# Axe--/Visual-Question-Answering

Hardware: AMD Instinct MI355X
Metric: QA-pairs/sec (train step, attention model, K=1000) (higher is better)
Workload: dtype f32

## Files before the change

include/coattn.h:

```cpp
#ifndef COATTN_H
#define COATTN_H

#include <stddef.h>
#include <stdint.h>

#ifdef __cplusplus
extern "C" {
#endif

#define COATTN_F32 0
#define COATTN_BF16 1

#define COATTN_IMPL_AUTO 0
#define COATTN_IMPL_GENERAL 1
#define COATTN_IMPL_FUSED 2
#define COATTN_FLAG_BF16_PROJ 4
#define COATTN_FLAG_BF16_IN 8
#define COATTN_FLAG_EXACT3 16
#define COATTN_FLAG_SPLIT2 32
#define COATTN_FLAG_F16PAIR 64
#define COATTN_FLAG_FAST16 128
#define COATTN_FLAG_BILINEAR 256
typedef struct coattn_params {
  const void* W_v; const void* b_v;
// ... 145 lines not shown
                         const void* g_loss, const void* g_logits, void* const* dv, void* const* dq,
                         const coattn_head_param_grads* pg, int accumulate, void* ws, int B, int d, int mlp, int K,
                         int dtype, int flags, void* stream);

#define COATTN_LOSS_SOFT_CE 1
#define COATTN_LOSS_BCE 2
int coattn_soft_loss_forward(const void* logits, const void* ans_idx, const void* ans_score, int A, int kind,
                             void* loss, void* dlogits, void* ws, int B, int K, int dtype, void* stream);
int coattn_vqa_score(const void* logits, const void* ans_idx, const void* ans_score, int A,
                     void* pred, void* row_score, void* score_sum,
                     void* ws, int B, int K, int dtype, void* stream);
int coattn_head_forward_soft(const void* const* v, const void* const* q, const coattn_head_params* p,
                             const void* ans_idx, const void* ans_score, int A, int kind,
                             void* logits, void* loss, void* saved, int B, int d, int mlp, int K, int dtype, int flags,
                             void* stream);

typedef struct coattn_adam_tensor {
  void* p; const void* g; void* m; void* v; int64_t n;
} coattn_adam_tensor;
size_t coattn_adam_workspace_bytes(const coattn_adam_tensor* t, int n_tensors);
int coattn_adam_step(const coattn_adam_tensor* t, int n_tensors, int step, double lr, double beta1, double beta2,
                     double eps, double weight_decay, double max_grad_norm, void* norm_out, void* ws, size_t ws_bytes,
                     void* stream);

int coattn_bn_supported(int B, int H, int W, int C, int pool, int dtype);
size_t coattn_bn_workspace_bytes(int B, int H, int W, int C);
int coattn_bn_relu_pool_forward(const void* x, const void* gamma, const void* beta, const void* conv_bias,
                                void* running_mean, void* running_var, double momentum, double eps, void* y,
                                void* stats_out, void* ws, int B, int H, int W, int C, int pool, int relu, int dtype,
                                void* stream);

int coattn_relu_pool_forward(const void* x, void* y, int B, int H, int W, int C, int dtype, void* stream);


typedef struct coattn_gemm_desc {
  const void* A; const void* B; const void* Cin; void* C;
  const void* bias_n; const void* bias_m;
  int M, N, K, batch, inner, inner_total, ksplit, act;
  float beta;
  int64_t a_sm, a_sk, a_sz, a_si, a_mdiv, a_sdiv;
  int64_t b_sk, b_sn, b_sz, b_si;
  int64_t c_sm, c_sn, c_sz, c_mdiv, c_sdiv;
  int64_t cin_sm, cin_sn, cin_sz, cin_mdiv, cin_sdiv;
  const void* a_ptrs[8]; const void* b_ptrs[8]; void* c_ptrs[8]; const void* cin_ptrs[8];
  int ptr_by_inner; int b_imod;
  int kband_n; int kband_lo[3]; int kband_hi[3];
  float out_scale;
} coattn_gemm_desc;

int coattn_gemm_f32(const coattn_gemm_desc* g, void* stream);

size_t coattn_linear_workspace_bytes(int N, int K);
int coattn_linear_forward(const void* x, int64_t ld_x, const void* W, const void* bias, void* y, void* wimg,
                          int M, int N, int K, float out_scale, int flags, void* stream);

size_t coattn_linear_wgrad_workspace_bytes(int n_out, int n_in);
int coattn_linear_weight_grad(const void* dy, int64_t ld_dy, const void* x, int64_t ld_x, void* dW, void* ws, int M,
                              int n_out, int n_in, int accumulate, void* stream);

int coattn_gemm_bf16(const coattn_gemm_desc* g, void* stream);

int coattn_p2p_enable_peer(int peer_device);
int coattn_p2p_reduce_scatter(const void* const* peer_bufs, int world, int rank, int64_t shard_elems, float scale,
                              void* stream);
int coattn_p2p_all_gather(const void* const* peer_bufs, int world, int rank, int64_t shard_elems, void* stream);

// ... 5 lines not shown
```

visual-question-answering_amd/_lib.py:

```python
from __future__ import annotations

import ctypes as C
import os
import subprocess

_HERE = os.path.dirname(os.path.abspath(__file__))
LIB_PATH = os.environ.get("COATTN_LIB_PATH") or os.path.join(_HERE, "libcoattn_hip.so")
CSRC = os.path.join(_HERE, "csrc")

EXPORTS = ("coattn_version", "coattn_last_error", "coattn_fused_supported", "coattn_workspace_bytes",
           "coattn_forward", "coattn_attention_forward", "coattn_backward", "coattn_gemm_f32", "coattn_gemm_bf16",
           "coattn_phrase_workspace_bytes", "coattn_phrase_forward", "coattn_phrase_backward",
           "coattn_ce_workspace_bytes", "coattn_ce_forward", "coattn_linear_workspace_bytes", "coattn_linear_forward",
           "coattn_linear_wgrad_workspace_bytes", "coattn_linear_weight_grad",
           "coattn_head_workspace_bytes", "coattn_head_forward", "coattn_head_backward", "coattn_head_status",
           "coattn_ce_status", "coattn_p2p_enable_peer", "coattn_p2p_reduce_scatter", "coattn_p2p_all_gather",
           "coattn_profile_begin", "coattn_profile_end", "coattn_features_native", "coattn_status",
           "coattn_phrase_status", "coattn_status_accumulate", "coattn_phrase_status_accumulate", "coattn_infer",
           "coattn_forward_len", "coattn_infer_len", "coattn_attention_forward_len", "coattn_backward_len",
           "coattn_forward_maps", "coattn_forward_maps_len", "coattn_backward_maps", "coattn_backward_maps_len",
           "coattn_alt_workspace_bytes", "coattn_alt_forward", "coattn_alt_backward",
           "coattn_soft_loss_forward", "coattn_vqa_score", "coattn_head_forward_soft",
           "coattn_adam_workspace_bytes", "coattn_adam_step",
           "coattn_bn_supported", "coattn_bn_workspace_bytes", "coattn_bn_relu_pool_forward", "coattn_relu_pool_forward")

F32 = 0
BF16 = 1
IMPL_AUTO, IMPL_GENERAL, IMPL_FUSED = 0, 1, 2
FLAG_BF16_PROJ = 4
FLAG_BF16_IN = 8
FLAG_EXACT3 = 16
FLAG_SPLIT2 = 32
FLAG_F16PAIR = 64
FLAG_FAST16 = 128
LOSS_SOFT_CE, LOSS_BCE = 1, 2
MAX_ANSWERS = 16
LOSS_KINDS = {"soft_ce": LOSS_SOFT_CE, "bce": LOSS_BCE}
FLAG_BILINEAR = 256


def precision_flag(fast: bool) -> int:
    return FLAG_FAST16 if fast else 0


def default_fast() -> bool:
    return os.environ.get("VQA_PRECISION", "exact") == "fast"


class Params(C.Structure):
    _fields_ = [(n, C.c_void_p) for n in ("W_v", "b_v", "W_q", "b_q", "w_v", "c_v", "w_q", "c_q", "W_b", "b_b")]


class ParamGrads(C.Structure):
    _fields_ = [(n, C.c_void_p) for n in ("dW_v", "db_v", "dW_q", "db_q", "dw_v", "dc_v", "dw_q", "dc_q", "dW_b", "db_b")]


ALT_PARAM_NAMES = ("W_x1", "b_x1", "w_h1", "c_h1", "W_x2", "b_x2", "W_g2", "b_g2", "w_h2", "c_h2",
# ... 192 lines not shown
    lib.coattn_linear_workspace_bytes.restype = C.c_size_t
    lib.coattn_linear_forward.argtypes = ([C.c_void_p, C.c_int64] + [C.c_void_p] * 4 + [C.c_int] * 3
                                          + [C.c_float, C.c_int, C.c_void_p])
    lib.coattn_linear_wgrad_workspace_bytes.argtypes = [C.c_int, C.c_int]
    lib.coattn_linear_wgrad_workspace_bytes.restype = C.c_size_t
    lib.coattn_linear_weight_grad.argtypes = ([C.c_void_p, C.c_int64, C.c_void_p, C.c_int64, C.c_void_p, C.c_void_p]
                                              + [C.c_int] * 4 + [C.c_void_p])
    lib.coattn_ce_status.argtypes = [C.c_void_p, C.c_int, C.c_void_p]
    lib.coattn_status.argtypes = [C.c_void_p] + [C.c_int] * 6 + [C.c_void_p, C.POINTER(C.c_float)]
    lib.coattn_phrase_status.argtypes = [C.c_void_p] + [C.c_int] * 3 + [C.c_void_p, C.POINTER(C.c_float)]
    lib.coattn_status_accumulate.argtypes = [C.c_void_p] + [C.c_int] * 6 + [C.c_void_p, C.c_void_p]
    lib.coattn_phrase_status_accumulate.argtypes = [C.c_void_p] + [C.c_int] * 3 + [C.c_void_p, C.c_void_p]
    lib.coattn_p2p_enable_peer.argtypes = [C.c_int]
    lib.coattn_p2p_reduce_scatter.argtypes = [C.POINTER(C.c_void_p), C.c_int, C.c_int, C.c_int64, C.c_float, C.c_void_p]
    lib.coattn_p2p_all_gather.argtypes = [C.POINTER(C.c_void_p), C.c_int, C.c_int, C.c_int64, C.c_void_p]
    lib.coattn_profile_begin.argtypes = [C.c_void_p]
    lib.coattn_profile_end.argtypes = [C.POINTER(C.c_float), C.c_char_p, C.c_int, C.c_int]
    lib.coattn_features_native.argtypes = [C.c_void_p, C.c_int, C.c_int64, C.c_int64, C.c_int64, C.c_void_p,
                                           C.c_int, C.c_int, C.c_int, C.c_void_p]
    lib.coattn_head_status.argtypes = [C.c_void_p] + [C.c_int] * 4 + [C.c_void_p]
    lib.coattn_head_workspace_bytes.argtypes = [C.c_int] * 5 + [C.POINTER(C.c_size_t)] * 2
    lib.coattn_soft_loss_forward.argtypes = [C.c_void_p] * 3 + [C.c_int] * 2 + [C.c_void_p] * 3 + [C.c_int] * 3 + [C.c_void_p]
    lib.coattn_vqa_score.argtypes = [C.c_void_p] * 3 + [C.c_int] + [C.c_void_p] * 4 + [C.c_int] * 3 + [C.c_void_p]
    lib.coattn_adam_workspace_bytes.argtypes = [C.POINTER(AdamTensor), C.c_int]
    lib.coattn_adam_workspace_bytes.restype = C.c_size_t
    lib.coattn_adam_step.argtypes = ([C.POINTER(AdamTensor), C.c_int, C.c_int] + [C.c_double] * 6
                                     + [C.c_void_p, C.c_void_p, C.c_size_t, C.c_void_p])
    lib.coattn_bn_supported.argtypes = [C.c_int] * 6
    lib.coattn_bn_workspace_bytes.argtypes = [C.c_int] * 4
    lib.coattn_bn_workspace_bytes.restype = C.c_size_t
    lib.coattn_bn_relu_pool_forward.argtypes = ([C.c_void_p] * 6 + [C.c_double] * 2 + [C.c_void_p] * 3 + [C.c_int] * 7
                                                + [C.c_void_p])
    lib.coattn_relu_pool_forward.argtypes = [C.c_void_p] * 2 + [C.c_int] * 5 + [C.c_void_p]
    _lib = lib
    return lib


class RangeError(FloatingPointError):
    """An operand of the tolerance mode (FLAG_FAST16) left the exact range of its two FP16 pieces: the call's results are
    clamped, not within tolerance of the reference.  Use the exact mode (the modules' default; Trainer(precision="exact"))."""


F16_EXACT = 65504.0

_pending = []
_range_acc = {}


def note_status(kind: str, buf, dims, dev) -> None:
    import torch
    _pending.append((kind, buf, dims, dev, torch.cuda.current_stream(dev).cuda_stream))
    if not torch.cuda.is_current_stream_capturing():
        fold_range()


def _acc(dev):
    import torch
    key = dev.index if dev.index is not None else torch.cuda.current_device()
    a = _range_acc.get(key)
    if a is None:
        a = _range_acc[key] = torch.zeros(2, device=dev, dtype=torch.float32)
    return a


def fold_range() -> None:
    lib = load()
# ... 99 lines not shown
```

visual-question-answering_amd/csrc/api.hip:

```cpp
#include "common.h"
#include "fused.h"

#include <string.h>

static thread_local char g_err[512] = "";

void coattn_set_error(const char* fmt, ...) {
  va_list ap;
  va_start(ap, fmt);
  vsnprintf(g_err, sizeof(g_err), fmt, ap);
  va_end(ap);
}

extern "C" int coattn_version(void) { return 1400; }

namespace {
constexpr int kProfMax = 48;
struct Prof {
  bool on = false;
  int n = 0, created = 0;
  hipEvent_t ev[kProfMax + 1];
  const char* name[kProfMax];
};
thread_local Prof g_prof;
}

void prof_mark(hipStream_t s, const char* name) {
  Prof& p = g_prof;
  if (!p.on || p.n >= kProfMax) return;
  if (hipEventRecord(p.ev[p.n + 1], s) != hipSuccess) { p.on = false; return; }
  p.name[p.n++] = name;
}

extern "C" int coattn_profile_begin(void* stream) {
  Prof& p = g_prof;
  while (p.created <= kProfMax) {
    if (hipEventCreate(&p.ev[p.created]) != hipSuccess) { coattn_set_error("profile: hipEventCreate failed"); return -3; }
    ++p.created;
  }
  p.n = 0;
  if (hipEventRecord(p.ev[0], (hipStream_t)stream) != hipSuccess) { coattn_set_error("profile: hipEventRecord failed"); return -3; }
  p.on = true;
  return 0;
}

extern "C" int coattn_profile_end(float* us, char* names, int names_bytes, int max_marks) {
  Prof& p = g_prof;
// ... 818 lines not shown
```

visual-question-answering_amd/csrc/encoder.hip:

```cpp
#include <math.h>

#include "common.h"

namespace {

constexpr int kThreads = 256;
constexpr int kMaxStatBlocks = 2048;
constexpr int kPixelsPerStatBlock = 400;
constexpr int kMaxNormBlocks = 4096;
constexpr int kStatLoads = 8;

typedef double f64x2 __attribute__((ext_vector_type(2)));

inline int stat_blocks(int64_t pixels) {
  const int64_t g = pixels / kPixelsPerStatBlock;
  return g < 1 ? 1 : g > kMaxStatBlocks ? kMaxStatBlocks : (int)g;
}

inline size_t partial_bytes(int G, int C) { return (size_t)G * C * sizeof(f64x2); }

__global__ __launch_bounds__(kThreads) void bn_stats_partial_kernel(const f32x4* __restrict__ x, f64x2* __restrict__ partial,
                                                                    int64_t total4, int c4) {
  __shared__ double sh[8][kThreads];
  const int tid = threadIdx.x;
// ... 57 lines not shown
    const f64x2 p = partial[(int64_t)g * C + c];
    s += p.x;
    q += p.y;
  }
  sh[0][tid] = s;
  sh[1][tid] = q;
  for (int w = kThreads / 2; w >= 4; w >>= 1) {
    __syncthreads();
    if (tid < w) {
      s += sh[0][tid + w];
      q += sh[1][tid + w];
      sh[0][tid] = s;
      sh[1][tid] = q;
    }
  }
  if (tid >= 4) return;
  const double mean = s / count;
  double var = q / count - mean * mean;
  var = var < 0.0 ? 0.0 : var;
  const float mean_hi = (float)mean;
  ws_f[c] = mean_hi;
  ws_f[C + c] = (float)(mean - (double)mean_hi);
  ws_f[2 * C + c] = (float)((double)gamma[c] / sqrt(var + eps));
  ws_f[3 * C + c] = (float)var;
  const double bias = conv_bias ? (double)conv_bias[c] : 0.0;
  running_mean[c] = (float)((1.0 - momentum) * (double)running_mean[c] + momentum * (mean + bias));
  running_var[c] = (float)((1.0 - momentum) * (double)running_var[c] + momentum * (var * (count / (count - 1.0))));
  if (stats_out) {
    stats_out[c] = mean_hi;
    stats_out[C + c] = (float)var;
  }
}

struct Affine {
  float mean[4], lo[4], scale[4], beta[4];
};

__device__ __forceinline__ f32x4 affine(const f32x4 v, const Affine& a) {
  f32x4 t;
#pragma unroll
  for (int e = 0; e < 4; ++e) t[e] = fmaf((v[e] - a.mean[e]) - a.lo[e], a.scale[e], a.beta[e]);
  return t;
}
__device__ __forceinline__ f32x4 max_nan(const f32x4 a, const f32x4 b) {
  f32x4 m;
#pragma unroll
  for (int e = 0; e < 4; ++e) m[e] = (a[e] > b[e] || a[e] != a[e]) ? a[e] : b[e];
  return m;
}
__device__ __forceinline__ f32x4 relu_nan(const f32x4 a) {
  f32x4 r;
#pragma unroll
  for (int e = 0; e < 4; ++e) r[e] = a[e] < 0.f ? 0.f : a[e];
  return r;
}

template <bool POOL, bool AFFINE = true>
__global__ __launch_bounds__(kThreads) void bn_relu_pool_kernel(const f32x4* __restrict__ x, const float* __restrict__ ws_f,
                                                                const float* __restrict__ beta, f32x4* __restrict__ y,
                                                                int H, int W, int C, int c4_shift, int64_t total4, int relu) {
  const int tid = threadIdx.x;
  const int c4 = C >> 2;
  const int cg = tid & (c4 - 1);
  Affine a;
#pragma unroll
  for (int e = 0; e < 4; ++e) {
    a.mean[e] = AFFINE ? ws_f[4 * cg + e] : 0.f;
    a.lo[e] = AFFINE ? ws_f[C + 4 * cg + e] : 0.f;
    a.scale[e] = AFFINE ? ws_f[2 * C + 4 * cg + e] : 1.f;
    a.beta[e] = AFFINE ? beta[4 * cg + e] : 0.f;
  }
  const int64_t stride = (int64_t)gridDim.x * kThreads;
  int64_t o = (int64_t)blockIdx.x * kThreads + tid;
  if (!POOL) {
    for (; o < total4; o += 4 * stride) {
      f32x4 v[4];
#pragma unroll
      for (int u = 0; u < 4; ++u)
        if (o + u * stride < total4) v[u] = x[o + u * stride];
#pragma unroll
      for (int u = 0; u < 4; ++u)
        if (o + u * stride < total4) {
          const f32x4 t = affine(v[u], a);
          y[o + u * stride] = relu ? relu_nan(t) : t;
        }
    }
    return;
  }
  const uint32_t Ho = (uint32_t)H >> 1, Wo = (uint32_t)W >> 1;
  const int64_t row4 = (int64_t)W * c4;
  for (; o < total4; o += 2 * stride) {
    f32x4 v[2][4];
    bool live[2];
#pragma unroll
    for (int u = 0; u < 2; ++u) {
      const int64_t ou = o + u * stride;
      live[u] = ou < total4;
      if (live[u]) {
        const uint32_t pix = (uint32_t)(ou >> c4_shift);
        const uint32_t wo = pix % Wo, r = pix / Wo, ho = r % Ho, b = r / Ho;
        const int64_t in4 = (((int64_t)b * H + 2 * ho) * W + 2 * wo) * c4 + cg;
        v[u][0] = x[in4];
        v[u][1] = x[in4 + c4];
        v[u][2] = x[in4 + row4];
        v[u][3] = x[in4 + row4 + c4];
      }
    }
#pragma unroll
    for (int u = 0; u < 2; ++u)
      if (live[u]) {
        const f32x4 t = AFFINE ? max_nan(max_nan(affine(v[u][0], a), affine(v[u][1], a)),
                                         max_nan(affine(v[u][2], a), affine(v[u][3], a)))
                               : max_nan(max_nan(v[u][0], v[u][1]), max_nan(v[u][2], v[u][3]));
        y[o + u * stride] = relu ? relu_nan(t) : t;
      }
  }
}

inline int log2_exact(int v) {
  int s = 0;
  while ((1 << s) < v) ++s;
  return s;
}

}

extern "C" int coattn_bn_supported(int B, int H, int W, int C, int pool, int dtype) {
  if (dtype != COATTN_F32 || B < 1 || H < 1 || W < 1) return 0;
  if (C < 16 || C > 512 || (C & (C - 1)) != 0) return 0;
  const int64_t limit = (int64_t)1 << 31;
  const int64_t bh = (int64_t)B * H;
  if (bh >= limit) return 0;
  const int64_t pixels = bh * W;
  if (pixels < 2 || pixels >= limit || pixels * C >= limit) return 0;
  if (pool && (H < 2 || W < 2)) return 0;
  return 1;
}

extern "C" size_t coattn_bn_workspace_bytes(int B, int H, int W, int C) {
  if (!coattn_bn_supported(B, H, W, C, 0, COATTN_F32)) {
    coattn_set_error("bn_workspace_bytes: B=%d H=%d W=%d C=%d is not a supported shape (coattn_bn_supported)", B, H, W, C);
    return 0;
  }
  return partial_bytes(stat_blocks((int64_t)B * H * W), C) + (size_t)4 * C * sizeof(float);
}
// ... 3 lines not shown
                                           void* stats_out, void* ws, int B, int H, int W, int C, int pool, int relu,
                                           int dtype, void* stream) {
  CA_CHECK_ARG(B >= 1 && H >= 1 && W >= 1 && C >= 1, "bn_relu_pool_forward: B=%d H=%d W=%d C=%d (all must be >= 1)", B, H, W,
               C);
  CA_CHECK_ARG(coattn_bn_supported(B, H, W, C, pool, dtype),
               "bn_relu_pool_forward: B=%d H=%d W=%d C=%d pool=%d dtype=%d is not supported (coattn_bn_supported)", B, H, W, C,
               pool, dtype);
  CA_CHECK_ARG(x && gamma && beta && running_mean && running_var && y && ws,
               "bn_relu_pool_forward: a null x / gamma / beta / running_mean / running_var / y / ws");
  CA_CHECK_ARG(((reinterpret_cast<uintptr_t>(x) | reinterpret_cast<uintptr_t>(y) | reinterpret_cast<uintptr_t>(ws)) & 15) == 0,
               "bn_relu_pool_forward: x, y and ws must be 16-byte aligned");
  CA_CHECK_ARG(x != y, "bn_relu_pool_forward: y must not be x");
  CA_CHECK_ARG(momentum >= 0.0 && momentum <= 1.0, "bn_relu_pool_forward: momentum %g outside [0, 1]", momentum);
  CA_CHECK_ARG(eps > 0.0, "bn_relu_pool_forward: eps %g (must be > 0)", eps);
  hipStream_t s = (hipStream_t)stream;
  const int c4 = C / 4;
  const int64_t pixels = (int64_t)B * H * W;
  const int G = stat_blocks(pixels);
  f64x2* partial = (f64x2*)ws;
  float* ws_f = (float*)((char*)ws + partial_bytes(G, C));
  hipLaunchKernelGGL(bn_stats_partial_kernel, dim3(G), dim3(kThreads), 0, s, (const f32x4*)x, partial, pixels * c4, c4);
  CA_CHECK_LAUNCH("bn_stats_partial");
  hipLaunchKernelGGL(bn_finalize_kernel, dim3(c4), dim3(kThreads), 0, s, (const f64x2*)partial, G, C, (double)pixels,
                     (const float*)gamma, (const float*)conv_bias, (float*)running_mean, (float*)running_var, momentum, eps,
                     ws_f, (float*)stats_out);
  CA_CHECK_LAUNCH("bn_finalize");
  const int64_t out_pixels = pool ? (int64_t)B * (H / 2) * (W / 2) : pixels;
  const int64_t total4 = out_pixels * c4;
  const int per_thread = pool ? 2 : 4;
  int64_t blocks = (total4 + (int64_t)kThreads * per_thread - 1) / ((int64_t)kThreads * per_thread);
  if (blocks > kMaxNormBlocks) blocks = kMaxNormBlocks;
  if (pool)
    hipLaunchKernelGGL(bn_relu_pool_kernel<true>, dim3((unsigned)blocks), dim3(kThreads), 0, s, (const f32x4*)x, ws_f,
                       (const float*)beta, (f32x4*)y, H, W, C, log2_exact(c4), total4, relu);
  else
    hipLaunchKernelGGL(bn_relu_pool_kernel<false>, dim3((unsigned)blocks), dim3(kThreads), 0, s, (const f32x4*)x, ws_f,
                       (const float*)beta, (f32x4*)y, H, W, C, log2_exact(c4), total4, relu);
  CA_CHECK_LAUNCH("bn_relu_pool");
  prof_mark(s, "bn_relu_pool");
  return 0;
}

extern "C" int coattn_relu_pool_forward(const void* x, void* y, int B, int H, int W, int C, int dtype, void* stream) {
  CA_CHECK_ARG(B >= 1 && H >= 1 && W >= 1 && C >= 1, "relu_pool_forward: B=%d H=%d W=%d C=%d (all must be >= 1)", B, H, W, C);
  CA_CHECK_ARG(coattn_bn_supported(B, H, W, C, 1, dtype),
               "relu_pool_forward: B=%d H=%d W=%d C=%d dtype=%d is not supported (coattn_bn_supported with pool)", B, H, W, C,
               dtype);
  CA_CHECK_ARG(x && y, "relu_pool_forward: a null x / y");
  CA_CHECK_ARG(((reinterpret_cast<uintptr_t>(x) | reinterpret_cast<uintptr_t>(y)) & 15) == 0,
               "relu_pool_forward: x and y must be 16-byte aligned");
  CA_CHECK_ARG(x != y, "relu_pool_forward: y must not be x");
  hipStream_t s = (hipStream_t)stream;
  const int c4 = C / 4;
  const int64_t total4 = (int64_t)B * (H / 2) * (W / 2) * c4;
  int64_t blocks = (total4 + (int64_t)kThreads * 2 - 1) / ((int64_t)kThreads * 2);
  if (blocks > kMaxNormBlocks) blocks = kMaxNormBlocks;
  hipLaunchKernelGGL((bn_relu_pool_kernel<true, false>), dim3((unsigned)blocks), dim3(kThreads), 0, s, (const f32x4*)x,
                     (const float*)nullptr, (const float*)nullptr, (f32x4*)y, H, W, C, log2_exact(c4), total4, 1);
  CA_CHECK_LAUNCH("relu_pool");
  prof_mark(s, "relu_pool");
  return 0;
}
```

visual-question-answering_amd/encoder.py:

```python
from __future__ import annotations

import ctypes as C
import os

import torch
import torch.nn as nn

from . import _lib


def _pair(v):
    return tuple(v) if isinstance(v, (tuple, list)) else (v, v)


def pool_is_2x2(pool: nn.MaxPool2d) -> bool:
    stride = pool.kernel_size if pool.stride is None else pool.stride
    return (_pair(pool.kernel_size) == (2, 2) and _pair(stride) == (2, 2) and _pair(pool.padding) == (0, 0)
            and _pair(pool.dilation) == (1, 1) and not pool.ceil_mode and not pool.return_indices)


def mode() -> str:
    return {"0": "stock", "1": "bn"}.get(os.environ.get("VQA_ENCODER_FUSED", ""), "pool")


def relu_pool_fusable(pool: nn.MaxPool2d, x: torch.Tensor) -> bool:
    if mode() == "stock" or not pool_is_2x2(pool) or (torch.is_grad_enabled() and x.requires_grad):
        return False
    if not (x.is_cuda and x.dtype == torch.float32 and x.dim() == 4 and x.is_contiguous(memory_format=torch.channels_last)):
        return False
    B, Ch, H, W = x.shape
    return bool(_lib.load().coattn_bn_supported(B, H, W, Ch, 1, _lib.F32))


def relu_pool(x: torch.Tensor) -> torch.Tensor:
    B, Ch, H, W = x.shape
    if not (x.is_cuda and x.dtype == torch.float32 and x.is_contiguous(memory_format=torch.channels_last)):
        raise ValueError("relu_pool: needs a CUDA fp32 channels_last [B,C,H,W] tensor, got %s %s strides %s"
                         % (tuple(x.shape), x.dtype, x.stride()))
    y = torch.empty((B, Ch, H // 2, W // 2), device=x.device, dtype=torch.float32, memory_format=torch.channels_last)
    with _lib.on_device(x.device):
        _lib.check(_lib.load().coattn_relu_pool_forward(_lib.ptr(x), _lib.ptr(y), B, H, W, Ch, _lib.F32,
                                                        C.c_void_p(_lib.stream_ptr(x.device))), "coattn_relu_pool_forward")
    return y


def modules_fusable(conv: nn.Conv2d, bn: nn.BatchNorm2d, pool, x: torch.Tensor) -> bool:
    if mode() != "bn" or not x.is_cuda:
        return False
    if not (bn.training and bn.affine and bn.track_running_stats and bn.momentum is not None and bn.running_mean is not None):
        return False
    params = (conv.weight, conv.bias, bn.weight, bn.bias)
    if torch.is_grad_enabled() and (x.requires_grad or any(p is not None and p.requires_grad for p in params)):
        return False
    if conv.padding_mode != "zeros":
        return False
    b = conv.bias
    if b is not None and (b.requires_grad or b.dtype != torch.float32 or b.device != x.device or not b.is_contiguous()):
        return False
    return pool is None or pool_is_2x2(pool)


def output_fusable(z: torch.Tensor, bn: nn.BatchNorm2d, pool: bool) -> bool:
    if not (z.is_cuda and z.dtype == torch.float32 and z.dim() == 4 and z.is_contiguous(memory_format=torch.channels_last)):
        return False
    for t in (bn.weight, bn.bias, bn.running_mean, bn.running_var):
        if t.dtype != torch.float32 or t.device != z.device or not t.is_contiguous():
            return False
    B, Ch, H, W = z.shape
    return bool(_lib.load().coattn_bn_supported(B, H, W, Ch, int(pool), _lib.F32))


def bn_relu_pool(x: torch.Tensor, bn: nn.BatchNorm2d, conv_bias=None, pool: bool = False, stats_out=None) -> torch.Tensor:
    lib = _lib.load()
    B, Ch, H, W = x.shape
    for t, shape in ((conv_bias, (Ch,)), (stats_out, (2, Ch))):
        if t is not None and not (t.dtype == torch.float32 and t.device == x.device and t.is_contiguous()
                                  and tuple(t.shape) == shape):
            raise ValueError("bn_relu_pool: conv_bias / stats_out must be contiguous fp32 [C] / [2, C] tensors on x's device")
    if not output_fusable(x, bn, pool):
        raise ValueError("bn_relu_pool: needs a CUDA fp32 channels_last [B,C,H,W] tensor of a shape coattn_bn_supported "
                         "takes, got %s %s strides %s" % (tuple(x.shape), x.dtype, x.stride()))
    Ho, Wo = (H // 2, W // 2) if pool else (H, W)
    y = torch.empty((B, Ch, Ho, Wo), device=x.device, dtype=torch.float32, memory_format=torch.channels_last)
    ws = torch.empty((lib.coattn_bn_workspace_bytes(B, H, W, Ch) + 3) // 4, device=x.device, dtype=torch.float32)
    with torch.no_grad(), _lib.on_device(x.device):
        rc = lib.coattn_bn_relu_pool_forward(_lib.ptr(x), _lib.ptr(bn.weight), _lib.ptr(bn.bias), _lib.ptr(conv_bias),
                                             _lib.ptr(bn.running_mean), _lib.ptr(bn.running_var), float(bn.momentum),
                                             float(bn.eps), _lib.ptr(y), _lib.ptr(stats_out), _lib.ptr(ws), B, H, W, Ch,
                                             int(pool), 1, _lib.F32, C.c_void_p(_lib.stream_ptr(x.device)))
        _lib.check(rc, "coattn_bn_relu_pool_forward")
        if bn.num_batches_tracked is not None:
            bn.num_batches_tracked.add_(1)
    return y
```

visual-question-answering_amd/modules.py:

```python
from __future__ import annotations

import os
from collections import OrderedDict

import torch
import torch.nn as nn
import torch.nn.functional as F
from torch.nn.utils.rnn import pack_padded_sequence, pad_packed_sequence

from . import encoder
from .alternating import AlternatingCoAttention
from .coattention import ParallelCoAttention
from .head import answer_head

_VGG11_CFG = (64, "M", 128, "M", 256, 256, "M", 512, 512, "M", 512, 512, "M")


def vgg11_bn_features() -> nn.Sequential:
    mods, c_in = [], 3
    for item in _VGG11_CFG:
        if item == "M":
            mods.append(nn.MaxPool2d(2, 2))
            continue
        mods.extend((nn.Conv2d(c_in, item, 3, padding=1), nn.BatchNorm2d(item), nn.ReLU(inplace=True)))
        c_in = item
    return nn.Sequential(*mods)


def _vgg11_bn_classifier_head() -> list:
    return [nn.Linear(512 * 7 * 7, 4096), nn.ReLU(True), nn.Dropout(), nn.Linear(4096, 4096), nn.ReLU(True),
            nn.Dropout()]


def _load_vgg_weights(features: nn.Module, classifier: nn.Module | None, weights_path):
    if not weights_path or not os.path.isfile(str(weights_path)):
        return False
    sd = torch.load(weights_path, map_location="cpu")
    features.load_state_dict({k[len("features."):]: v for k, v in sd.items() if k.startswith("features.")})
    if classifier is not None:
        cls = {k[len("classifier."):]: v for k, v in sd.items() if k.startswith("classifier.")}
        classifier.load_state_dict({k: v for k, v in cls.items() if not k.startswith("6.")}, strict=False)
    return True


def run_conv_bn_stack(seq: nn.Sequential, x: torch.Tensor) -> torch.Tensor:
    mods = list(seq)
    if os.environ.get("VQA_ENCODER_REWRITE", "1") == "0":
        return seq(x)
    i, n = 0, len(mods)
    while i < n:
        m = mods[i]
        nxt = mods[i + 1] if i + 1 < n else None
        pool = mods[i + 3] if i + 3 < n and isinstance(mods[i + 3], nn.MaxPool2d) else None
        fuse = (isinstance(m, nn.Conv2d) and isinstance(nxt, nn.BatchNorm2d) and i + 2 < n and isinstance(mods[i + 2], nn.ReLU)
                and encoder.modules_fusable(m, nxt, pool, x))
        if (isinstance(m, nn.Conv2d) and (fuse or (m.bias is not None and not m.bias.requires_grad)) and m.padding_mode == "zeros"
                and isinstance(nxt, nn.BatchNorm2d) and nxt.training and nxt.momentum is not None):
            x = F.conv2d(x, m.weight, None, m.stride, m.padding, m.dilation, m.groups)
            if fuse and encoder.output_fusable(x, nxt, pool is not None):
                x = encoder.bn_relu_pool(x, nxt, conv_bias=m.bias, pool=pool is not None)
                i += 3 if pool is None else 4
                continue
            x = nxt(x)
            if m.bias is not None and nxt.track_running_stats and nxt.running_mean is not None:
                with torch.no_grad():
                    nxt.running_mean.add_(m.bias.to(nxt.running_mean.dtype), alpha=nxt.momentum)
            i += 2
        elif isinstance(m, nn.ReLU) and isinstance(nxt, nn.MaxPool2d):
            x = encoder.relu_pool(x) if encoder.relu_pool_fusable(nxt, x) else F.relu(nxt(x), inplace=True)
            i += 2
        else:
            x = m(x)
            i += 1
    return x


class ImageCoAttentionEncoder(nn.Module):

    def __init__(self, is_trainable, weights_path):
        super().__init__()
        self.is_trainable = is_trainable
        self.weights_path = weights_path
        self.vgg11_encoder = vgg11_bn_features()
        _load_vgg_weights(self.vgg11_encoder, None, weights_path)
        self.flatten = nn.Flatten(start_dim=2, end_dim=3)
        if not is_trainable:
            for prm in self.vgg11_encoder.parameters():
                prm.requires_grad = False

    def forward(self, x_img):
        grid = self.flatten(run_conv_bn_stack(self.vgg11_encoder, x_img))
        return grid.permute(0, 2, 1)


class _Bottleneck(nn.Module):

    def __init__(self, c_in, width, stride, downsample):
        super().__init__()
        self.conv1 = nn.Conv2d(c_in, width, 1, bias=False); self.bn1 = nn.BatchNorm2d(width)
        self.conv2 = nn.Conv2d(width, width, 3, stride=stride, padding=1, bias=False); self.bn2 = nn.BatchNorm2d(width)
# ... 306 lines not shown
```

Before: 6468.

## Add bit-exact MIOpen-matching BatchNorm forward fused with ReLU and max-pool

Adds HIP kernels that reproduce MIOpen's BatchNorm training statistics reduction: a partial-sum stats kernel followed by a finalize kernel. Those statistics feed the existing affine, ReLU and optional 2x2 max-pool kernel through a new STOCK affine variant. In the encoder's 'pool' mode, conv+BN+ReLU(+pool) groups are routed to this path. Each shape is first verified bit-for-bit against the stock chain and falls back to it on any mismatch. The aim is to remove the separate BN output, ReLU and pool passes over the activations while keeping results identical. The cost is a one-time verification run per shape, plus extra launches for the stats and finalize kernels.

```diff
diff --git a/include/coattn.h b/include/coattn.h
--- a/include/coattn.h
+++ b/include/coattn.h
@@ -201,6 +201,12 @@
 
 int coattn_relu_pool_forward(const void* x, void* y, int B, int H, int W, int C, int dtype, void* stream);
 
+int coattn_bn_exact_geometry(int B, int H, int W, int C, int dtype, int* out);
+size_t coattn_bn_exact_workspace_bytes(int B, int H, int W, int C);
+int coattn_bn_exact_forward(const void* x, const void* gamma, const void* beta, void* running_mean, void* running_var,
+                            double momentum, double eps, void* y, void* save_mean, void* save_invstd, void* ws, int B, int H,
+                            int W, int C, int pool, int relu, int dtype, void* stream);
+
 
 typedef struct coattn_gemm_desc {
   const void* A; const void* B; const void* Cin; void* C;
diff --git a/visual-question-answering_amd/_lib.py b/visual-question-answering_amd/_lib.py
--- a/visual-question-answering_amd/_lib.py
+++ b/visual-question-answering_amd/_lib.py
@@ -22,7 +22,8 @@
            "coattn_alt_workspace_bytes", "coattn_alt_forward", "coattn_alt_backward",
            "coattn_soft_loss_forward", "coattn_vqa_score", "coattn_head_forward_soft",
            "coattn_adam_workspace_bytes", "coattn_adam_step",
-           "coattn_bn_supported", "coattn_bn_workspace_bytes", "coattn_bn_relu_pool_forward", "coattn_relu_pool_forward")
+           "coattn_bn_supported", "coattn_bn_workspace_bytes", "coattn_bn_relu_pool_forward", "coattn_relu_pool_forward",
+           "coattn_bn_exact_geometry", "coattn_bn_exact_workspace_bytes", "coattn_bn_exact_forward")
 
 F32 = 0
 BF16 = 1
@@ -281,6 +282,11 @@
     lib.coattn_bn_relu_pool_forward.argtypes = ([C.c_void_p] * 6 + [C.c_double] * 2 + [C.c_void_p] * 3 + [C.c_int] * 7
                                                 + [C.c_void_p])
     lib.coattn_relu_pool_forward.argtypes = [C.c_void_p] * 2 + [C.c_int] * 5 + [C.c_void_p]
+    lib.coattn_bn_exact_geometry.argtypes = [C.c_int] * 5 + [C.POINTER(C.c_int)]
+    lib.coattn_bn_exact_workspace_bytes.argtypes = [C.c_int] * 4
+    lib.coattn_bn_exact_workspace_bytes.restype = C.c_size_t
+    lib.coattn_bn_exact_forward.argtypes = ([C.c_void_p] * 5 + [C.c_double] * 2 + [C.c_void_p] * 4 + [C.c_int] * 7
+                                            + [C.c_void_p])
     _lib = lib
     return lib
 
diff --git a/visual-question-answering_amd/csrc/api.hip b/visual-question-answering_amd/csrc/api.hip
--- a/visual-question-answering_amd/csrc/api.hip
+++ b/visual-question-answering_amd/csrc/api.hip
@@ -12,7 +12,7 @@
   va_end(ap);
 }
 
-extern "C" int coattn_version(void) { return 1400; }
+extern "C" int coattn_version(void) { return 1500; }
 
 namespace {
 constexpr int kProfMax = 48;
diff --git a/visual-question-answering_amd/csrc/encoder.hip b/visual-question-answering_amd/csrc/encoder.hip
--- a/visual-question-answering_amd/csrc/encoder.hip
+++ b/visual-question-answering_amd/csrc/encoder.hip
@@ -113,14 +113,115 @@
   }
 }
 
+struct BnGeom {
+  int vec, g0, g1, g2, nel, ngrps, ngrps2, f0, f1, f2;
+};
+constexpr int kGeomInts = 10;
+constexpr int kExactLoads = 8;
+
+__device__ __forceinline__ void acc_miopen(f32x4& sum, f32x4& sq, const f32x4 v) {
+#pragma unroll
+  for (int e = 0; e < 4; ++e) {
+    sum[e] += v[e];
+    sq[e] = __builtin_fmaf(v[e], v[e], sq[e]);
+  }
+}
+
+__device__ __forceinline__ void tree_miopen(f32x4& sum, f32x4& sq, float scale, f32x4* lds, int xs, int xl, int yl, int size) {
+  const int o1 = 2 * (xl + yl * xs);
+  lds[o1] = sum;
+  lds[o1 + 1] = sq;
+  __syncthreads();
+  for (int red = size >> 1; red > 0; red >>= 1) {
+    if (yl < red) {
+      const int o2 = o1 + red * xs * 2;
+      sum += lds[o2];
+      sq += lds[o2 + 1];
+      lds[o1] = sum;
+      lds[o1 + 1] = sq;
+    }
+    __syncthreads();
+  }
+  sum = lds[2 * xl] * scale;
+  sq = lds[2 * xl + 1] * scale;
+}
+
+__global__ __launch_bounds__(1024) void bn_stats_miopen_kernel(const f32x4* __restrict__ x, f32x4* __restrict__ partial, BnGeom g,
+                                                               int B, int HW, int c4) {
+  extern __shared__ f32x4 lds_stats[];
+  const int xl = threadIdx.x, yl = threadIdx.y + threadIdx.z * g.g1;
+  const int xg = blockIdx.x * g.g0 + xl, yg = blockIdx.y * g.g1 + threadIdx.y, zg = blockIdx.z * g.g2 + threadIdx.z;
+  f32x4 sum = {0.f, 0.f, 0.f, 0.f}, sq = {0.f, 0.f, 0.f, 0.f};
+  const int n0 = zg * g.nel;
+  if (yg < HW && n0 < B) {
+    const int64_t sample4 = (int64_t)HW * c4;
+    const f32x4* p = x + ((int64_t)n0 * sample4 + (int64_t)yg * c4 + xg);
+    const int nel = B - n0 < g.nel ? B - n0 : g.nel;
+    int n = 0;
+    for (; n + kExactLoads <= nel; n += kExactLoads) {
+      f32x4 v[kExactLoads];
+#pragma unroll
+      for (int u = 0; u < kExactLoads; ++u) v[u] = p[(n + u) * sample4];
+#pragma unroll
+      for (int u = 0; u < kExactLoads; ++u) acc_miopen(sum, sq, v[u]);
+    }
+    for (; n < nel; ++n) acc_miopen(sum, sq, p[n * sample4]);
+  }
+  tree_miopen(sum, sq, 1.f, lds_stats, g.g0, xl, yl, g.g1 * g.g2);
+  if (yl == 0) {
+    f32x4* out = partial + (((int64_t)blockIdx.z * g.ngrps + blockIdx.y) * c4 + xg) * 2;
+    out[0] = sum;
+    out[1] = sq;
+  }
+}
+
+__global__ __launch_bounds__(1024) void bn_finalize_miopen_kernel(const f32x4* __restrict__ partial, BnGeom g, int c4, float inhw,
+                                                                  float unbias, float factor, float eps, f32x4* running_mean,
+                                                                  f32x4* running_var, f32x4* __restrict__ save_mean,
+                                                                  f32x4* __restrict__ save_invstd) {
+  extern __shared__ f32x4 lds_final[];
+  const int xl = threadIdx.x, yl = threadIdx.y + threadIdx.z * g.f1;
+  const int xg = blockIdx.x * g.f0 + xl;
+  f32x4 mean = {0.f, 0.f, 0.f, 0.f}, var = {0.f, 0.f, 0.f, 0.f};
+  for (int z = threadIdx.z; z < g.ngrps2; z += g.f2)
+    for (int y = threadIdx.y; y < g.ngrps; y += g.f1) {
+      const f32x4* p = partial + (((int64_t)z * g.ngrps + y) * c4 + xg) * 2;
+      mean += p[0];
+      var += p[1];
+    }
+  tree_miopen(mean, var, inhw, lds_final, g.f0, xl, yl, g.f1 * g.f2);
+  f32x4 invstd;
+#pragma unroll
+  for (int e = 0; e < 4; ++e) {
+    var[e] = __builtin_fmaxf(__builtin_fmaf(-mean[e], mean[e], var[e]), 0.f);
+    invstd[e] = __builtin_amdgcn_rsqf(var[e] + eps);
+  }
+  if (yl != 0) return;
+  const f32x4 rm = running_mean[xg], rv = running_var[xg];
+  f32x4 nm, nv;
+#pragma unroll
+  for (int e = 0; e < 4; ++e) {
+    nm[e] = __builtin_fmaf(mean[e], factor, __builtin_fmaf(-factor, rm[e], rm[e]));
+    const float adjust = var[e] * unbias;
+    nv[e] = __builtin_fmaf(1.f - factor, rv[e], factor * adjust);
+  }
+  running_mean[xg] = nm;
+  running_var[xg] = nv;
+  save_mean[xg] = mean;
+  save_invstd[xg] = invstd;
+}
+
 struct Affine {
-  float mean[4], lo[4], scale[4], beta[4];
+  float mean[4], lo[4], scale[4], beta[4], gamma[4];
 };
 
+template <bool STOCK>
 __device__ __forceinline__ f32x4 affine(const f32x4 v, const Affine& a) {
   f32x4 t;
 #pragma unroll
-  for (int e = 0; e < 4; ++e) t[e] = fmaf((v[e] - a.mean[e]) - a.lo[e], a.scale[e], a.beta[e]);
+  for (int e = 0; e < 4; ++e)
+    t[e] = STOCK ? __builtin_fmaf(a.gamma[e], (v[e] - a.mean[e]) * a.scale[e], a.beta[e])
+                 : fmaf((v[e] - a.mean[e]) - a.lo[e], a.scale[e], a.beta[e]);
   return t;
 }
 __device__ __forceinline__ f32x4 max_nan(const f32x4 a, const f32x4 b) {
@@ -136,8 +237,9 @@
   return r;
 }
 
-template <bool POOL, bool AFFINE = true>
+template <bool POOL, bool AFFINE = true, bool STOCK = false>
 __global__ __launch_bounds__(kThreads) void bn_relu_pool_kernel(const f32x4* __restrict__ x, const float* __restrict__ ws_f,
+                                                                const float* __restrict__ scale, const float* __restrict__ gamma,
                                                                 const float* __restrict__ beta, f32x4* __restrict__ y,
                                                                 int H, int W, int C, int c4_shift, int64_t total4, int relu) {
   const int tid = threadIdx.x;
@@ -147,8 +249,9 @@
 #pragma unroll
   for (int e = 0; e < 4; ++e) {
     a.mean[e] = AFFINE ? ws_f[4 * cg + e] : 0.f;
-    a.lo[e] = AFFINE ? ws_f[C + 4 * cg + e] : 0.f;
-    a.scale[e] = AFFINE ? ws_f[2 * C + 4 * cg + e] : 1.f;
+    a.lo[e] = AFFINE && !STOCK ? ws_f[C + 4 * cg + e] : 0.f;
+    a.scale[e] = AFFINE ? scale[4 * cg + e] : 1.f;
+    a.gamma[e] = STOCK ? gamma[4 * cg + e] : 1.f;
     a.beta[e] = AFFINE ? beta[4 * cg + e] : 0.f;
   }
   const int64_t stride = (int64_t)gridDim.x * kThreads;
@@ -162,7 +265,7 @@
 #pragma unroll
       for (int u = 0; u < 4; ++u)
         if (o + u * stride < total4) {
-          const f32x4 t = affine(v[u], a);
+          const f32x4 t = affine<STOCK>(v[u], a);
           y[o + u * stride] = relu ? relu_nan(t) : t;
         }
     }
@@ -190,8 +293,8 @@
 #pragma unroll
     for (int u = 0; u < 2; ++u)
       if (live[u]) {
-        const f32x4 t = AFFINE ? max_nan(max_nan(affine(v[u][0], a), affine(v[u][1], a)),
-                                         max_nan(affine(v[u][2], a), affine(v[u][3], a)))
+        const f32x4 t = AFFINE ? max_nan(max_nan(affine<STOCK>(v[u][0], a), affine<STOCK>(v[u][1], a)),
+                                         max_nan(affine<STOCK>(v[u][2], a), affine<STOCK>(v[u][3], a)))
                                : max_nan(max_nan(v[u][0], v[u][1]), max_nan(v[u][2], v[u][3]));
         y[o + u * stride] = relu ? relu_nan(t) : t;
       }
@@ -261,10 +364,10 @@
   if (blocks > kMaxNormBlocks) blocks = kMaxNormBlocks;
   if (pool)
     hipLaunchKernelGGL(bn_relu_pool_kernel<true>, dim3((unsigned)blocks), dim3(kThreads), 0, s, (const f32x4*)x, ws_f,
-                       (const float*)beta, (f32x4*)y, H, W, C, log2_exact(c4), total4, relu);
+                       ws_f + 2 * C, (const float*)nullptr, (const float*)beta, (f32x4*)y, H, W, C, log2_exact(c4), total4, relu);
   else
     hipLaunchKernelGGL(bn_relu_pool_kernel<false>, dim3((unsigned)blocks), dim3(kThreads), 0, s, (const f32x4*)x, ws_f,
-                       (const float*)beta, (f32x4*)y, H, W, C, log2_exact(c4), total4, relu);
+                       ws_f + 2 * C, (const float*)nullptr, (const float*)beta, (f32x4*)y, H, W, C, log2_exact(c4), total4, relu);
   CA_CHECK_LAUNCH("bn_relu_pool");
   prof_mark(s, "bn_relu_pool");
   return 0;
@@ -285,8 +388,106 @@
   int64_t blocks = (total4 + (int64_t)kThreads * 2 - 1) / ((int64_t)kThreads * 2);
   if (blocks > kMaxNormBlocks) blocks = kMaxNormBlocks;
   hipLaunchKernelGGL((bn_relu_pool_kernel<true, false>), dim3((unsigned)blocks), dim3(kThreads), 0, s, (const f32x4*)x,
-                     (const float*)nullptr, (const float*)nullptr, (f32x4*)y, H, W, C, log2_exact(c4), total4, 1);
+                     (const float*)nullptr, (const float*)nullptr, (const float*)nullptr, (const float*)nullptr, (f32x4*)y, H, W,
+                     C, log2_exact(c4), total4, 1);
   CA_CHECK_LAUNCH("relu_pool");
   prof_mark(s, "relu_pool");
   return 0;
 }
+
+namespace {
+
+constexpr int64_t kSmallMaxHWC = 153600, kLargeMinHWC = 163840;
+constexpr int kExactMaxB = 1024;
+
+bool bn_exact_geometry(int B, int H, int W, int C, int dtype, BnGeom* g) {
+  if (dtype != COATTN_F32 || !coattn_bn_supported(B, H, W, C, 0, dtype)) return false;
+  if (C < 64 || B > kExactMaxB) return false;
+  const int64_t hw = (int64_t)H * W, hwc = hw * C;
+  if (hwc > kSmallMaxHWC && hwc < kLargeMinHWC) return false;
+  g->vec = 4;
+  g->g0 = 16;
+  g->g1 = hwc <= kSmallMaxHWC ? 8 : 16;
+  g->g2 = 1;
+  g->nel = B;
+  g->ngrps = (int)((hw + g->g1 - 1) / g->g1);
+  g->ngrps2 = 1;
+  g->f0 = 2;
+  g->f1 = g->g0 * g->g1 / 2;
+  g->f2 = 1;
+  if (hw % g->g1 == 1) return false;
+  return g->ngrps <= 65535;
+}
+
+inline size_t exact_partial_bytes(const BnGeom& g, int C) { return (size_t)g.ngrps * g.ngrps2 * C * 2 * sizeof(float); }
+
+}
+
+extern "C" int coattn_bn_exact_geometry(int B, int H, int W, int C, int dtype, int* out) {
+  BnGeom g;
+  if (!bn_exact_geometry(B, H, W, C, dtype, &g)) return 0;
+  if (out) {
+    const int v[kGeomInts] = {g.vec, g.g0, g.g1, g.g2, g.nel, g.ngrps, g.ngrps2, g.f0, g.f1, g.f2};
+    for (int i = 0; i < kGeomInts; ++i) out[i] = v[i];
+  }
+  return kGeomInts;
+}
+
+extern "C" size_t coattn_bn_exact_workspace_bytes(int B, int H, int W, int C) {
+  BnGeom g;
+  if (!bn_exact_geometry(B, H, W, C, COATTN_F32, &g)) {
+    coattn_set_error("bn_exact_workspace_bytes: B=%d H=%d W=%d C=%d is not a covered shape (coattn_bn_exact_geometry)", B, H, W, C);
+    return 0;
+  }
+  return exact_partial_bytes(g, C);
+}
+
+extern "C" int coattn_bn_exact_forward(const void* x, const void* gamma, const void* beta, void* running_mean, void* running_var,
+                                       double momentum, double eps, void* y, void* save_mean, void* save_invstd, void* ws, int B,
+                                       int H, int W, int C, int pool, int relu, int dtype, void* stream) {
+  CA_CHECK_ARG(B >= 1 && H >= 1 && W >= 1 && C >= 1, "bn_exact_forward: B=%d H=%d W=%d C=%d (all must be >= 1)", B, H, W, C);
+  BnGeom g;
+  CA_CHECK_ARG(bn_exact_geometry(B, H, W, C, dtype, &g) && coattn_bn_supported(B, H, W, C, pool, dtype),
+               "bn_exact_forward: B=%d H=%d W=%d C=%d pool=%d dtype=%d is not a covered shape (coattn_bn_exact_geometry)", B, H,
+               W, C, pool, dtype);
+  CA_CHECK_ARG(x && gamma && beta && running_mean && running_var && y && save_mean && save_invstd && ws,
+               "bn_exact_forward: a null x / gamma / beta / running_mean / running_var / y / save_mean / save_invstd / ws");
+  CA_CHECK_ARG(((reinterpret_cast<uintptr_t>(x) | reinterpret_cast<uintptr_t>(y) | reinterpret_cast<uintptr_t>(ws) |
+                 reinterpret_cast<uintptr_t>(gamma) | reinterpret_cast<uintptr_t>(beta) | reinterpret_cast<uintptr_t>(running_mean) |
+                 reinterpret_cast<uintptr_t>(running_var) | reinterpret_cast<uintptr_t>(save_mean) |
+                 reinterpret_cast<uintptr_t>(save_invstd)) & 15) == 0,
+               "bn_exact_forward: every pointer must be 16-byte aligned");
+  CA_CHECK_ARG(x != y, "bn_exact_forward: y must not be x");
+  CA_CHECK_ARG(momentum >= 0.0 && momentum <= 1.0, "bn_exact_forward: momentum %g outside [0, 1]", momentum);
+  CA_CHECK_ARG(eps > 0.0, "bn_exact_forward: eps %g (must be > 0)", eps);
+  hipStream_t s = (hipStream_t)stream;
+  const int c4 = C / 4, hw = H * W;
+  const int64_t pixels = (int64_t)B * hw;
+  f32x4* partial = (f32x4*)ws;
+  hipLaunchKernelGGL(bn_stats_miopen_kernel, dim3(c4 / g.g0, g.ngrps, g.ngrps2), dim3(g.g0, g.g1, g.g2),
+                     (size_t)2 * g.g0 * g.g1 * g.g2 * sizeof(f32x4), s, (const f32x4*)x, partial, g, B, hw, c4);
+  CA_CHECK_LAUNCH("bn_stats_miopen");
+  const float n_f = (float)pixels;
+  const float inhw = (float)(1.0 / (double)pixels), unbias = pixels == 1 ? 1.f : n_f / (n_f - 1.f);
+  hipLaunchKernelGGL(bn_finalize_miopen_kernel, dim3(c4 / g.f0), dim3(g.f0, g.f1, g.f2),
+                     (size_t)2 * g.f0 * g.f1 * g.f2 * sizeof(f32x4), s, (const f32x4*)partial, g, c4, inhw, unbias,
+                     (float)momentum, (float)eps, (f32x4*)running_mean, (f32x4*)running_var, (f32x4*)save_mean,
+                     (f32x4*)save_invstd);
+  CA_CHECK_LAUNCH("bn_finalize_miopen");
+  const int64_t out_pixels = pool ? (int64_t)B * (H / 2) * (W / 2) : pixels;
+  const int64_t total4 = out_pixels * c4;
+  const int per_thread = pool ? 2 : 4;
+  int64_t blocks = (total4 + (int64_t)kThreads * per_thread - 1) / ((int64_t)kThreads * per_thread);
+  if (blocks > kMaxNormBlocks) blocks = kMaxNormBlocks;
+  if (pool)
+    hipLaunchKernelGGL((bn_relu_pool_kernel<true, true, true>), dim3((unsigned)blocks), dim3(kThreads), 0, s, (const f32x4*)x,
+                       (const float*)save_mean, (const float*)save_invstd, (const float*)gamma, (const float*)beta, (f32x4*)y, H,
+                       W, C, log2_exact(c4), total4, relu);
+  else
+    hipLaunchKernelGGL((bn_relu_pool_kernel<false, true, true>), dim3((unsigned)blocks), dim3(kThreads), 0, s, (const f32x4*)x,
+                       (const float*)save_mean, (const float*)save_invstd, (const float*)gamma, (const float*)beta, (f32x4*)y, H,
+                       W, C, log2_exact(c4), total4, relu);
+  CA_CHECK_LAUNCH("bn_relu_pool_exact");
+  prof_mark(s, "bn_exact");
+  return 0;
+}
diff --git a/visual-question-answering_amd/encoder.py b/visual-question-answering_amd/encoder.py
--- a/visual-question-answering_amd/encoder.py
+++ b/visual-question-answering_amd/encoder.py
@@ -2,6 +2,7 @@
 
 import ctypes as C
 import os
+import warnings
 
 import torch
 import torch.nn as nn
@@ -45,7 +46,19 @@
 
 
 def modules_fusable(conv: nn.Conv2d, bn: nn.BatchNorm2d, pool, x: torch.Tensor) -> bool:
-    if mode() != "bn" or not x.is_cuda:
+    return mode() == "bn" and _group_fusable(conv, bn, pool, x)
+
+
+def exact_enabled() -> bool:
+    return mode() == "pool" and os.environ.get("VQA_ENCODER_EXACT_BN", "1") != "0"
+
+
+def exact_modules_fusable(conv: nn.Conv2d, bn: nn.BatchNorm2d, pool, x: torch.Tensor) -> bool:
+    return exact_enabled() and not torch.is_autocast_enabled() and _group_fusable(conv, bn, pool, x)
+
+
+def _group_fusable(conv: nn.Conv2d, bn: nn.BatchNorm2d, pool, x: torch.Tensor) -> bool:
+    if not x.is_cuda:
         return False
     if not (bn.training and bn.affine and bn.track_running_stats and bn.momentum is not None and bn.running_mean is not None):
         return False
@@ -92,3 +105,91 @@
         if bn.num_batches_tracked is not None:
             bn.num_batches_tracked.add_(1)
     return y
+
+
+GEOMETRY_FIELDS = ("vec", "g0", "g1", "g2", "samples_per_thread", "pixel_groups", "sample_groups", "f0", "f1", "f2")
+_exact = {}
+
+
+def exact_geometry(B: int, H: int, W: int, Ch: int):
+    out = (C.c_int * len(GEOMETRY_FIELDS))()
+    n = _lib.load().coattn_bn_exact_geometry(B, H, W, Ch, _lib.F32, out)
+    return dict(zip(GEOMETRY_FIELDS, out)) if n == len(GEOMETRY_FIELDS) else None
+
+
+def exact_output_fusable(z: torch.Tensor, bn: nn.BatchNorm2d, pool: bool) -> bool:
+    if not output_fusable(z, bn, pool) or exact_geometry(z.shape[0], z.shape[2], z.shape[3], z.shape[1]) is None:
+        return False
+    return all(t.data_ptr() % 16 == 0 for t in (z, bn.weight, bn.bias, bn.running_mean, bn.running_var))
+
+
+def exact_report() -> dict:
+    return {k: dict(v) for k, v in _exact.items()}
+
+
+def _bn_exact_raw(x, weight, bias, running_mean, running_var, momentum, eps, pool: bool):
+    lib = _lib.load()
+    B, Ch, H, W = x.shape
+    Ho, Wo = (H // 2, W // 2) if pool else (H, W)
+    y = torch.empty((B, Ch, Ho, Wo), device=x.device, dtype=torch.float32, memory_format=torch.channels_last)
+    save = torch.empty((2, Ch), device=x.device, dtype=torch.float32)
+    ws = torch.empty((lib.coattn_bn_exact_workspace_bytes(B, H, W, Ch) + 3) // 4, device=x.device, dtype=torch.float32)
+    with torch.no_grad(), _lib.on_device(x.device):
+        rc = lib.coattn_bn_exact_forward(_lib.ptr(x), _lib.ptr(weight), _lib.ptr(bias), _lib.ptr(running_mean),
+                                         _lib.ptr(running_var), float(momentum), float(eps), _lib.ptr(y), _lib.ptr(save[0]),
+                                         _lib.ptr(save[1]), _lib.ptr(ws), B, H, W, Ch, int(pool), 1, _lib.F32,
+                                         C.c_void_p(_lib.stream_ptr(x.device)))
+        _lib.check(rc, "coattn_bn_exact_forward")
+    return y, save[0], save[1]
+
+
+def bn_exact(x: torch.Tensor, bn: nn.BatchNorm2d, pool: bool = False) -> torch.Tensor:
+    if not exact_output_fusable(x, bn, pool):
+        raise ValueError("bn_exact: needs a CUDA fp32 channels_last [B,C,H,W] tensor of a shape coattn_bn_exact_geometry "
+                         "covers, got %s %s strides %s" % (tuple(x.shape), x.dtype, x.stride()))
+    y, _, _ = _bn_exact_raw(x, bn.weight, bn.bias, bn.running_mean, bn.running_var, bn.momentum, bn.eps, pool)
+    if bn.num_batches_tracked is not None:
+        with torch.no_grad():
+            bn.num_batches_tracked.add_(1)
+    return y
+
+
+def _stock_chain(x: torch.Tensor, bn: nn.BatchNorm2d, pool) -> torch.Tensor:
+    z = bn(x)
+    if pool is None:
+        return torch.relu_(z)
+    return relu_pool(z) if relu_pool_fusable(pool, z) else torch.relu_(pool(z))
+
+
+def _differs(a: torch.Tensor, b: torch.Tensor) -> torch.Tensor:
+    return ~((a == b) | (a.isnan() & b.isnan())).all()
+
+
+def _verify(x: torch.Tensor, bn: nn.BatchNorm2d, pool, key) -> torch.Tensor:
+    with torch.no_grad():
+        rm0, rv0 = bn.running_mean.clone(), bn.running_var.clone()
+        y = _stock_chain(x, bn, pool)
+        _, save_mean, save_invstd = torch.miopen_batch_norm(x, bn.weight, bn.bias, rm0.clone(), rv0.clone(), True,
+                                                            bn.momentum, bn.eps)
+        mine_y, mine_mean, mine_invstd = _bn_exact_raw(x, bn.weight, bn.bias, rm0, rv0, bn.momentum, bn.eps, pool is not None)
+        names = ("y", "running_mean", "running_var", "save_mean", "save_invstd")
+        pairs = ((mine_y, y), (rm0, bn.running_mean), (rv0, bn.running_var), (mine_mean, save_mean), (mine_invstd, save_invstd))
+        flags = torch.stack([_differs(a, b) for a, b in pairs]).tolist()
+    first = next((n for n, f in zip(names, flags) if f), None)
+    B, Ch, H, W = x.shape
+    _exact[key] = {"verified": first is None, "first_difference": first, "geometry": exact_geometry(B, H, W, Ch)}
+    if first is not None:
+        warnings.warn("encoder: bn_exact does not reproduce the stock BatchNorm for B=%d C=%d H=%d W=%d pool=%d (%s differs); "
+                      "this shape stays on the stock kernels" % (B, Ch, H, W, int(pool is not None), first))
+    return y
+
+
+def bn_exact_or_stock(x: torch.Tensor, bn: nn.BatchNorm2d, pool) -> torch.Tensor:
+    B, Ch, H, W = x.shape
+    key = (x.device.index if x.device.index is not None else torch.cuda.current_device(), B, Ch, H, W, pool is not None)
+    state = _exact.get(key)
+    if state is None:
+        if torch.cuda.is_current_stream_capturing():
+            return _stock_chain(x, bn, pool)
+        return _verify(x, bn, pool, key)
+    return bn_exact(x, bn, pool is not None) if state["verified"] else _stock_chain(x, bn, pool)
diff --git a/visual-question-answering_amd/modules.py b/visual-question-answering_amd/modules.py
--- a/visual-question-answering_amd/modules.py
+++ b/visual-question-answering_amd/modules.py
@@ -52,20 +52,22 @@
         m = mods[i]
         nxt = mods[i + 1] if i + 1 < n else None
         pool = mods[i + 3] if i + 3 < n and isinstance(mods[i + 3], nn.MaxPool2d) else None
-        fuse = (isinstance(m, nn.Conv2d) and isinstance(nxt, nn.BatchNorm2d) and i + 2 < n and isinstance(mods[i + 2], nn.ReLU)
-                and encoder.modules_fusable(m, nxt, pool, x))
-        if (isinstance(m, nn.Conv2d) and (fuse or (m.bias is not None and not m.bias.requires_grad)) and m.padding_mode == "zeros"
-                and isinstance(nxt, nn.BatchNorm2d) and nxt.training and nxt.momentum is not None):
+        group = isinstance(m, nn.Conv2d) and isinstance(nxt, nn.BatchNorm2d) and i + 2 < n and isinstance(mods[i + 2], nn.ReLU)
+        fuse = group and encoder.modules_fusable(m, nxt, pool, x)
+        exact = group and encoder.exact_modules_fusable(m, nxt, pool, x)
+        if (isinstance(m, nn.Conv2d) and (fuse or exact or (m.bias is not None and not m.bias.requires_grad))
+                and m.padding_mode == "zeros" and isinstance(nxt, nn.BatchNorm2d) and nxt.training and nxt.momentum is not None):
             x = F.conv2d(x, m.weight, None, m.stride, m.padding, m.dilation, m.groups)
             if fuse and encoder.output_fusable(x, nxt, pool is not None):
                 x = encoder.bn_relu_pool(x, nxt, conv_bias=m.bias, pool=pool is not None)
                 i += 3 if pool is None else 4
                 continue
-            x = nxt(x)
+            exact = exact and encoder.exact_output_fusable(x, nxt, pool is not None)
+            x = encoder.bn_exact_or_stock(x, nxt, pool) if exact else nxt(x)
             if m.bias is not None and nxt.track_running_stats and nxt.running_mean is not None:
                 with torch.no_grad():
                     nxt.running_mean.add_(m.bias.to(nxt.running_mean.dtype), alpha=nxt.momentum)
-            i += 2
+            i += 2 if not exact else 3 if pool is None else 4
         elif isinstance(m, nn.ReLU) and isinstance(nxt, nn.MaxPool2d):
             x = encoder.relu_pool(x) if encoder.relu_pool_fusable(nxt, x) else F.relu(nxt(x), inplace=True)
             i += 2
```

New measurement: 6964, median of 6. 1.08x the previous value.
